# karpathy/minbpe

Measured on AMD Instinct MI355X. Metric: BPE merges/sec, higher is better.
Workload: dtype int32; 1 GPU; regex1g: RegexTokenizer.train, 1 GB synth seed 2, vocab 32000; mode=default, parallelism=single

## Files before the change

### minbpe_amd/csrc/kernels/k_chain.hip

```cpp
#include <hip/hip_runtime.h>
#include <stdint.h>

#include "../bpe_device.h"

namespace bpe {
namespace BPE_G {

constexpr uint32_t CH_EX_CAP = 2048;

__device__ __forceinline__ int chain_match(const uint32_t *pa, const uint32_t *pb, uint32_t K, uint32_t w0, uint32_t w1) {
    const uint32_t x = w0 & IDMASK, y = w1 & NWMASK;
    int hit = -1;
    for (uint32_t p = 0; p < K; p++)
        if (x == pa[p] && y == pb[p]) hit = (int)p;
    return (w0 == INVALID_WORD) ? -1 : hit;
}

constexpr uint32_t CH_DCAP = 1024;
constexpr uint32_t CH_SD = 2 * CH_DCAP + 2;
__device__ __forceinline__ void chain_slot_load(const AbArgs &A, const uint32_t t, uint4 (&rv)[MJ], uint4 &hv) {
    const int lane = lane_id();
    const uint32_t *src = A.b0 + (size_t)t * TILE2;
#pragma unroll
    for (int j = 0; j < MJ; j++) rv[j] = *reinterpret_cast<const uint4 *>(src + j * 256 + lane * 4);
// ... 6 lines not shown
                                                 const uint32_t *pa, const uint32_t *pb, const uint32_t *pb1,
                                                 const uint32_t K, const uint32_t z0, const uint32_t brep,
                                                 uint4 (&rv)[MJ], const uint4 hv,
                                                 const uint32_t *ph = nullptr, const uint32_t hm = 0,
                                                 const uint32_t tl_in = 0xFFFFFFFFu) {
    const int lane = lane_id();
    const uint32_t Tl = tl_in != 0xFFFFFFFFu ? tl_in : min(A.T, A.st->tlive);
    const uint32_t *src;
    const uint32_t meta = bcast(hv.w, 2);
    const uint32_t len = meta & 0x7FFFFFFFu, buf = meta >> 31;
    auto keep_header = [&]() {
        if (DENSE && (lane == 2 || lane == 3)) reinterpret_cast<uint4 *>(A.hdr_out)[2 * (size_t)t + (lane - 2)] = hv;
    };
    if (len == 0) {
        keep_header();
        return;
    }
    if (buf) {
        src = A.b1 + (size_t)t * TILE2;
#pragma unroll
        for (int j = 0; j < MJ; j++) rv[j] = *reinterpret_cast<const uint4 *>(src + j * 256 + lane * 4);
    }
    const uint32_t first = bcast(hv.x, 2);
    uint32_t halo0 = bcast(hv.x, 4), halo1 = bcast(hv.y, 4), halo2 = bcast(hv.z, 4);
    uint32_t prev2 = bcast(hv.x, 1), prev1 = bcast(hv.y, 1);
    uint32_t tprev = t - 1;
    uint32_t tnext = t + 1;
    {
        const uint32_t nlen = bcast(hv.w, 4) & 0x7FFFFFFFu, plen = bcast(hv.w, 0) & 0x7FFFFFFFu;
        if ((t + 1 < Tl && nlen < 3) || (t > 0 && plen < 2)) {
            uint32_t ctx[7] = {0, 0, 0, 0, 0, 0, 0};
            if (lane == 0) slot_context_walk(A.hdr_in, t, Tl, ctx);
            halo0 = bcast(ctx[0], 0);
            halo1 = bcast(ctx[1], 0);
            halo2 = bcast(ctx[2], 0);
            prev2 = bcast(ctx[3], 0);
            prev1 = bcast(ctx[4], 0);
            tprev = bcast(ctx[5], 0);
            tnext = bcast(ctx[6], 0);
        }
    }
    auto at = [&](int q, uint32_t own) -> uint32_t {
        const int d = q - (int)len;
        return d < 0 ? own : (d == 0 ? halo0 : (d == 1 ? halo1 : (d == 2 ? halo2 : INVALID_WORD)));
    };
    uint32_t x[MJ][4];
#pragma unroll
    for (int j = 0; j < MJ; j++) {
        const int q0 = j * 256 + lane * 4;
        if ((j + 1) * 256 <= (int)len) {
            x[j][0] = rv[j].x;
            x[j][1] = rv[j].y;
            x[j][2] = rv[j].z;
            x[j][3] = rv[j].w;
        } else {
            x[j][0] = at(q0 + 0, rv[j].x);
            x[j][1] = at(q0 + 1, rv[j].y);
            x[j][2] = at(q0 + 2, rv[j].z);
            x[j][3] = at(q0 + 3, rv[j].w);
        }
    }
    uint32_t tail[3];
#pragma unroll
    for (int i = 0; i < 3; i++) tail[i] = at(TILE2 + i, 0u);
    uint32_t rb[MJ], jc[MJ], valid[MJ];
#pragma unroll
    for (int j = 0; j < MJ; j++) {
        rb[j] = 0;
        jc[j] = 0;
    }
    uint32_t s = 0;
    uint32_t ia[MJ];
#pragma unroll
    for (int j = 0; j < MJ; j++) ia[j] = 0;
    uint32_t ip = 0;
    if (hm) {
        auto code = [&](uint32_t w) -> uint32_t {
            const uint32_t id = w & IDMASK;
            const uint32_t e = ph[(__umul24(id, hm) >> 8) & 255u];
            return (e >> 8) == id ? (e & 255u) : 0u;
        };
#pragma unroll
        for (int j = 0; j < MJ; j++) {
#pragma unroll
            for (int k = 0; k < 4; k++) ia[j] |= code(x[j][k]) << (8 * k);
        }
        ip = code(prev1);
    } else {
        for (uint32_t p = 0; p < K; p++) {
            const uint32_t a = pa[p];
#pragma unroll
            for (int j = 0; j < MJ; j++) {
#pragma unroll
                for (int k = 0; k < 4; k++) ia[j] |= ((x[j][k] & IDMASK) == a) ? (p + 1u) << (8 * k) : 0u;
            }
            ip = ((prev1 & IDMASK) == a) ? p + 1u : ip;
        }
    }
#pragma unroll
    for (int j = 0; j < MJ; j++) {
        const uint32_t up = (j < MJ - 1) ? lane_first(x[(j + 1) % MJ][0]) : tail[0];
        const uint32_t nxw = lane_next(x[j][0], up);
#pragma unroll
        for (int k = 0; k < 4; k++) {
            const uint32_t nxt = (k < 3) ? x[j][k + 1] : nxw;
            const uint32_t i = (ia[j] >> (8 * k)) & 255u;
            const uint32_t m = (uint32_t)((nxt & NWMASK) == pb1[i]);
            rb[j] |= m << k;
            jc[j] |= (m ? i : 0u) << (8 * k);
        }
    }
    s = (uint32_t)((prev1 != INVALID_WORD) & ((first & NWMASK) == pb1[ip]));
#pragma unroll
    for (int j = 0; j < MJ; j++) {
        const int nb = (int)len - (j * 256 + lane * 4);
        valid[j] = nb >= 4 ? 0xFu : (nb <= 0 ? 0u : ((1u << nb) - 1u));
    }
    uint32_t anyr = 0;
#pragma unroll
    for (int j = 0; j < MJ; j++) anyr |= rb[j] & valid[j];
    const bool sites = __any(anyr != 0) != 0;
    if (!sites && !s) {
        keep_header();
        return;
    }
    uint32_t mb[MJ], kb[MJ], ex[MJ], cnt[MJ];
#pragma unroll
    for (int j = 0; j < MJ; j++) {
        mb[j] = rb[j] & valid[j];
        const uint32_t upr = (j > 0) ? ((lane_last(rb[(j + MJ - 1) % MJ]) >> 3) & 1u) : s;
        const uint32_t mp = (uint32_t)dpp_mov<0x138>((int)upr, (int)((rb[j] >> 3) & 1u));
        kb[j] = ~((mb[j] << 1) | mp) & valid[j] & 0xFu;
        cnt[j] = (uint32_t)__popc(kb[j]);
    }
    uint32_t total = 0;
    if constexpr (MJ == 4) {
        const uint32_t i01 = wave_iscan_add(cnt[0] | (cnt[1] << 16));
        const uint32_t i23 = wave_iscan_add(cnt[2] | (cnt[3] << 16));
        const uint32_t t01 = lane_last(i01), t23 = lane_last(i23);
        const uint32_t tot0 = t01 & 0xFFFFu, tot1 = t01 >> 16, tot2 = t23 & 0xFFFFu, tot3 = t23 >> 16;
        ex[0] = (i01 & 0xFFFFu) - cnt[0];
        ex[1] = tot0 + (i01 >> 16) - cnt[1];
        ex[2] = tot0 + tot1 + (i23 & 0xFFFFu) - cnt[2];
        ex[3] = tot0 + tot1 + tot2 + (i23 >> 16) - cnt[3];
        total = tot0 + tot1 + tot2 + tot3;
    } else {
#pragma unroll
        for (int j = 0; j < MJ; j++) {
            const uint32_t inc = wave_iscan_add(cnt[j]);
            ex[j] = total + inc - cnt[j];
            total += lane_last(inc);
        }
    }
    uint32_t fstore = 0;
    if (!s) {
        uint32_t fc = 0x7FFFFFFFu;
#pragma unroll
        for (int j = 0; j < MJ; j++) {
            if (mb[j]) {
                const uint32_t k0 = (uint32_t)__ffs((int)mb[j]) - 1u;
                fc = min(fc, ex[j] + (uint32_t)__popc(kb[j] & ((1u << k0) - 1u)));
            }
        }
        fstore = (uint32_t)wave_min_i32((int)fc) & ~3u;
    }
#pragma unroll
    for (int j = 0; j < MJ; j++) {
        uint32_t o = ex[j];
#pragma unroll
        for (int k = 0; k < 4; k++) {
            if ((kb[j] >> k) & 1u) {
                const uint32_t w = x[j][k];
                const uint32_t z = z0 + ((jc[j] >> (8 * k)) & 255u) - 1u;
                out[o++] = ((mb[j] >> k) & 1u) ? (z | (w & (FLAG | WMASK))) : w;
            }
        }
    }
    __builtin_amdgcn_fence(__ATOMIC_RELEASE, "wavefront");
    __builtin_amdgcn_wave_barrier();
    __builtin_amdgcn_fence(__ATOMIC_ACQUIRE, "wavefront");
    {
        uint32_t *dst = (buf ? A.b1 : A.b0) + (size_t)t * TILE2;
        for (uint32_t i = fstore + (uint32_t)lane * 4; i < total; i += 256)
            *reinterpret_cast<uint4 *>(dst + i) = *reinterpret_cast<const uint4 *>(&out[i]);
    }
    if (lane == 0) {
        uint32_t h[8];
        h[0] = total > 0 ? out[0] : INVALID_WORD;
        h[1] = total > 1 ? out[1] : INVALID_WORD;
        h[2] = total > 2 ? out[2] : INVALID_WORD;
        h[3] = total | (buf << 31);
        h[4] = total > 1 ? out[total - 2] : INVALID_WORD;
        h[5] = total > 0 ? out[total - 1] : INVALID_WORD;
        h[6] = h[7] = 0;
        if (DENSE) {
            reinterpret_cast<uint4 *>(A.hdr_out)[2 * (size_t)t] = make_uint4(h[0], h[1], h[2], h[3]);
            reinterpret_cast<uint4 *>(A.hdr_out)[2 * (size_t)t + 1] = make_uint4(h[4], h[5], 0u, 0u);
        } else {
            stage_put<THROUGH>(A.stage + t, t, h);
            atomicOr(&A.smask[t >> 5], 1u << (t & 31));
        }
        if (total < 3 && t + 1 < Tl) A.st->gap = 1;
    }
    if (!sites) return;
    const uint32_t vc = A.vcap & 0xFFFFFFu;
    uint32_t cm2 = 0, ct0 = 0, ct1 = 0;
    if (bcast(mb[0], 0) & 1u) cm2 = (uint32_t)(chain_match(pa, pb, K, prev2, prev1) + 1);
    const uint32_t cm1 = s ? ip : 0u;
    if (bcast(mb[MJ - 1], 63) & 0xCu) {
        ct0 = (uint32_t)(chain_match(pa, pb, K, tail[0], tail[1]) + 1);
        ct1 = (uint32_t)(chain_match(pa, pb, K, tail[1], tail[2]) + 1);
    }
#pragma unroll
    for (int j = 0; j < MJ; j++) {
        if (!__any(mb[j] != 0)) continue;
        uint32_t upm1, dn0;
        if (j > 0) upm1 = lane_last(x[(j + MJ - 1) % MJ][3]);
        else upm1 = prev1;
        if (j < MJ - 1) dn0 = lane_first(x[(j + 1) % MJ][0]);
        else dn0 = tail[0];
        uint32_t W[7];
        W[0] = (uint32_t)dpp_mov<0x138>((int)upm1, (int)x[j][3]);
        W[1] = x[j][0];
        W[2] = x[j][1];
        W[3] = x[j][2];
        W[4] = x[j][3];
        W[5] = lane_next(x[j][0], dn0);
        W[6] = lane_next(x[j][1], (j < MJ - 1) ? lane_first(x[(j + 1) % MJ][1]) : tail[1]);
        const uint32_t lo_fill = (j > 0) ? (lane_last(jc[(j + MJ - 1) % MJ]) >> 16) : (cm2 | (cm1 << 8));
        const uint32_t hi_fill = (j < MJ - 1) ? (lane_first(jc[(j + 1) % MJ]) & 0xFFFFu) : (ct0 | (ct1 << 8));
        const uint32_t lo = (uint32_t)dpp_mov<0x138>((int)lo_fill, (int)(jc[j] >> 16));
        const uint32_t hi = lane_next(jc[j] & 0xFFFFu, hi_fill);
        const unsigned long long win = (unsigned long long)lo | ((unsigned long long)jc[j] << 16) | ((unsigned long long)hi << 48);
        if (mb[j] == 0) continue;
        uint32_t todo = mb[j];
#pragma unroll
        for (int si = 0; si < 2; si++) {
            if (todo == 0) continue;
            const uint32_t k = (uint32_t)__ffs((int)todo) - 1u;
            todo &= todo - 1u;
            const int q = j * 256 + lane * 4 + (int)k;
            const unsigned long long wk = win >> (8u * k);
            const uint32_t p = ((uint32_t)(wk >> 16) & 255u) - 1u;
            const int li = (int)((uint32_t)wk & 255u) - 1, ri = (int)((uint32_t)(wk >> 32) & 255u) - 1;
            const uint32_t Z = z0 + p;
            uint32_t *dl, *dr;
            if (DENSE) {
                dl = sd + p * CH_SD;
                dr = dl + CH_DCAP;
                atomicAdd(&dl[2 * CH_DCAP + 1], 1u);
            } else {
                if (A.removed) atomicAdd(&A.removed[(p * (uint32_t)CH_RMV + (t & (uint32_t)(CH_RMV - 1))) * REMOVED_STRIDE], 1u);
                dl = A.delta + delta_rep_off(p * (uint32_t)CH_RSTRIDE + (t & (brep - 1u)), vc);
                dr = dl + vc;
            }
            const bool k1 = (k & 1u) != 0, k2 = (k & 2u) != 0;
            const uint32_t wa = k2 ? (k1 ? W[4] : W[3]) : (k1 ? W[2] : W[1]);
            const uint32_t wt = word_weight(wa);
            const uint32_t Lw = k2 ? (k1 ? W[3] : W[2]) : (k1 ? W[1] : W[0]);
            if (!(wa & FLAG) && Lw != INVALID_WORD) {
                if (li != (int)p) {
                    const uint32_t Lseq = (li >= 0 && (uint32_t)li < p) ? z0 + (uint32_t)li : (Lw & IDMASK);
                    atomicAdd(&dl[Lseq], wt);
                    if (!DENSE || A.idx) {
                        const uint32_t Lfin = li >= 0 ? z0 + (uint32_t)li : (Lw & IDMASK);
                        index_add(A.idx, A.istride, t, Lfin, Z);
                        if (q == 0) index_add(A.idx, A.istride, tprev, Lfin, Z);
                    }
                }
            }
            const uint32_t R = k2 ? (k1 ? W[6] : W[5]) : (k1 ? W[4] : W[3]);
            if (!(R & FLAG)) {
                if (ri == (int)p) {
                    if (DENSE) atomicAdd(&dl[2 * CH_DCAP], wt);
                    else atomicAdd(&A.st->badj[p], wt);
                } else {
                    atomicAdd(&dr[(ri >= 0 && (uint32_t)ri < p) ? z0 + (uint32_t)ri : (R & IDMASK)], wt);
                }
                if (!DENSE || A.idx) {
                    const uint32_t y = ri >= 0 ? z0 + (uint32_t)ri : (R & IDMASK);
                    index_add(A.idx, A.istride, t, Z, y);
                    if (q + 2 >= (int)len) index_add(A.idx, A.istride, tnext, Z, y);
                }
            }
        }
    }
}

__device__ __forceinline__ void merge_aa_wave(uint32_t *scr, const uint32_t t, const AbArgs &A, const ChainAa &X, const uint32_t a,
                                              const uint32_t newid, const uint32_t Tl) {
    const int lane = lane_id();
    uint32_t *s_hdr = scr, *s_halo = scr + 8;
    uint4 hv6 = (lane & 1) ? make_uint4(INVALID_WORD, INVALID_WORD, 0u, 0u) : make_uint4(INVALID_WORD, INVALID_WORD, INVALID_WORD, 0u);
    {
        const long long hi = 2ll * (long long)t - 2 + lane;
        if (lane < 6 && hi >= 0 && hi < 2ll * (long long)A.T) hv6 = reinterpret_cast<const uint4 *>(A.hdr_in)[hi];
    }
    const uint32_t mi = bcast(hv6.w, 2);
    const int len = (int)(mi & 0x7FFFFFFFu);
    if (len == 0) return;
    const uint32_t cur = mi >> 31;
    const uint32_t *src = (cur ? A.b1 : A.b0) + (size_t)t * TILE2;
    const uint32_t first = bcast(hv6.x, 2);
    uint32_t halo0 = bcast(hv6.x, 4), halo1 = bcast(hv6.y, 4), halo2 = bcast(hv6.z, 4);
    uint32_t prev1 = bcast(hv6.y, 1);
    uint32_t tnext = t + 1;
    {
        const uint32_t nlen = bcast(hv6.w, 4) & 0x7FFFFFFFu, plen = bcast(hv6.w, 0) & 0x7FFFFFFFu;
        if ((t + 1 < Tl && nlen < 3) || (t > 0 && plen < 2)) {
            uint32_t ctx[7] = {0, 0, 0, 0, 0, 0, 0};
            if (lane == 0) slot_context_walk(A.hdr_in, t, Tl, ctx);
            halo0 = bcast(ctx[0], 0);
            halo1 = bcast(ctx[1], 0);
            halo2 = bcast(ctx[2], 0);
            prev1 = bcast(ctx[4], 0);
            tnext = bcast(ctx[6], 0);
        }
    }
    const uint32_t hw1 = bcast(hv6.y, 2), hw2 = bcast(hv6.z, 2), hl0 = bcast(hv6.x, 3), hl1 = bcast(hv6.y, 3);
    if (lane == 0) {
        s_hdr[0] = first;
        s_hdr[1] = hw1;
        s_hdr[2] = hw2;
        s_hdr[3] = mi;
        s_hdr[4] = hl0;
        s_hdr[5] = hl1;
        s_halo[0] = halo0;
        s_halo[1] = halo1;
        s_halo[2] = halo2;
    }
    SlotRaw raw;
    slot_raw_load<true>(raw, src, len);
    __builtin_amdgcn_fence(__ATOMIC_RELEASE, "wavefront");
    __builtin_amdgcn_wave_barrier();
    __builtin_amdgcn_fence(__ATOMIC_ACQUIRE, "wavefront");
    Tile tl;
    tile_from_slot<true>(tl, raw, len, s_halo);
    tile_rbits(tl, a, a);
    uint32_t s = (uint32_t)((prev1 != INVALID_WORD) & ((prev1 & IDMASK) == a) & ((first & NWMASK) == a));
    {
        const unsigned long long tag = ((unsigned long long)(X.epoch & EPOCH_MASK)) << 42;
        uint32_t sc = 0;
        bool failed = false;
        if (s) {
            uint32_t u = t;
            uint32_t mu = 0;
            while (u-- > 0) {
                mu = A.hdr_in[u].meta;
                if (mu & 0x7FFFFFFFu) break;
            }
            const int lu = (int)(mu & 0x7FFFFFFFu);
            const uint32_t *pu = ((mu >> 31) ? A.b1 : A.b0) + (size_t)u * TILE2;
            int ones = 0;
            bool open = true;
            uint32_t nextw = first;
            for (int base = lu - 1; base >= 0 && open; base -= 64) {
                const int q = base - lane;
                const uint32_t xq = (q >= 0) ? pu[q] : INVALID_WORD;
                uint32_t nx = (uint32_t)__shfl_up((int)xq, 1);
                if (lane == 0) nx = nextw;
                const bool r = (q >= 0) && ((xq & IDMASK) == a) && ((nx & NWMASK) == a);
                const unsigned long long zeros = __ballot(!r);
                if (zeros) {
                    ones += __ffsll((long long)zeros) - 1;
                    const int zl = __ffsll((long long)zeros) - 1;
                    open = (base - zl < 0);
                    break;
                }
                ones += 64;
                nextw = (uint32_t)__shfl((int)xq, 63);
            }
            if (!open || ones < lu) {
                sc = (uint32_t)(ones & 1);
            } else {
                uint32_t su = 0;
                bool got = false;
                for (uint32_t spins = 0; spins < LOOKBACK_SPINS; spins++) {
                    const unsigned long long d = desc_load(&X.sdesc[u]);
                    if ((d >> 42) == (tag >> 42) + (1ull << 20)) {
                        su = (uint32_t)(d & 1u);
                        got = true;
                        break;
                    }
                    __builtin_amdgcn_s_sleep(8);
                }
                failed = !got;
                sc = (uint32_t)(((lu - 1) & 1) == 0) ^ su;
            }
        }
        if (lane == 0) {
            desc_store(&X.sdesc[t], tag | (1ull << 62) | sc);
            if (failed) atomicExch(&A.st->status, ST_LOOKBACK);
        }
        s = sc;
    }
    {
        uint32_t anyr = s;
        const int q0 = lane * 4;
        const int nb = len + 1 - q0;
        const uint32_t keep = nb >= 4 ? 0xFu : (nb <= 0 ? 0u : ((1u << nb) - 1u));
        anyr |= tl.rb[0] & keep;
        if (len == TILE2) anyr |= (uint32_t)(((tl.tail[0] & IDMASK) == a) & ((tl.tail[1] & NWMASK) == a));
        if (!__any(anyr != 0)) return;
    }
    tile_lzscan<true>(tl, nullptr);
    uint32_t kept = 0;
    bool changed = false;
    uint32_t *dst = (cur ? A.b0 : A.b1) + (size_t)t * TILE2;
    tile_rewrite<true, true, 1, true>(tl, s, a, a, newid, dst, nullptr, A.delta, A.vcap, len, &kept, &changed, s_hdr, A.idx,
                                      A.istride, t, tnext, t);
    __builtin_amdgcn_fence(__ATOMIC_RELEASE, "wavefront");
    __builtin_amdgcn_wave_barrier();
    __builtin_amdgcn_fence(__ATOMIC_ACQUIRE, "wavefront");
    if (lane == 0 && changed) {
        uint32_t h[8];
        h[0] = kept > 0 ? s_hdr[0] : INVALID_WORD;
        h[1] = kept > 1 ? s_hdr[1] : INVALID_WORD;
        h[2] = kept > 2 ? s_hdr[2] : INVALID_WORD;
        h[3] = kept | ((cur ^ 1u) << 31);
        h[4] = kept > 1 ? s_hdr[4] : INVALID_WORD;
        h[5] = kept > 0 ? s_hdr[5] : INVALID_WORD;
        h[6] = h[7] = 0;
        stage_put<false>(A.stage + t, t, h);
        atomicOr(&A.smask[t >> 5], 1u << (t & 31));
        atomicAdd(&X.removed[(t & 255u) * REMOVED_STRIDE], (uint32_t)len - kept);
        if (kept < 3 && t + 1 < Tl) A.st->gap = 1;
    }
    __builtin_amdgcn_fence(__ATOMIC_RELEASE, "wavefront");
    __builtin_amdgcn_wave_barrier();
}

__device__ __forceinline__ uint32_t chain_hash_find(const uint32_t *pa, uint32_t K, uint32_t *tab) {
    if (K < 5) return 0u;
    const uint32_t lane = (uint32_t)lane_id(), half = lane >> 5, l = lane & 31u;
    const bool in = l < K;
    const uint32_t a = in ? pa[l] : 0u;
// ... 741 lines not shown
```

### minbpe_amd/csrc/kernels/k_slots2.hip

```cpp
#include <hip/hip_runtime.h>
#include <stdint.h>

#include "../bpe_device.h"

namespace bpe {
namespace BPE_G {



__global__ void __launch_bounds__(256)
k_slot2_init(SlotHdr *__restrict__ hdr, uint64_t T, DevState *st, int par, uint32_t which,
             const uint32_t *__restrict__ ids) {
    const uint64_t n = st->n[par];
    if (blockIdx.x == 0 && threadIdx.x == 0) {
        st->gap = 0;
        st->tlive = (uint32_t)min(T, (n + TILE2 - 1) / TILE2);
    }
    const uint64_t stride = (uint64_t)gridDim.x * blockDim.x;
    for (uint64_t t = (uint64_t)blockIdx.x * blockDim.x + threadIdx.x; t < T; t += stride) {
        const uint64_t b0 = t * TILE2;
        const uint32_t len = b0 >= n ? 0u : (uint32_t)min((uint64_t)TILE2, n - b0);
        SlotHdr h;
        h.w0 = len > 0 ? ids[b0] : INVALID_WORD;
        h.w1 = len > 1 ? ids[b0 + 1] : INVALID_WORD;
// ... 31 lines not shown
    for (uint32_t u = t; u-- > 0 && got < 2;) {
        const SlotHdr hh = hdr[u];
        const uint32_t lu = hh.meta & 0x7FFFFFFFu;
        if (lu == 0) continue;
        if (got == 0) {
            p1 = hh.l1;
            tp = u;
            got = 1;
            if (lu >= 2) {
                p2 = hh.l0;
                got = 2;
            }
        } else {
            p2 = hh.l1;
            got = 2;
        }
    }
    ctx[0] = h0;
    ctx[1] = h1;
    ctx[2] = h2;
    ctx[3] = p2;
    ctx[4] = p1;
    ctx[5] = tp;
    ctx[6] = tn;
}

__device__ __forceinline__ uint32_t bcast(uint32_t v, int srclane) {
    return (uint32_t)__builtin_amdgcn_readlane((int)v, srclane);
}

template <bool SPARSE, bool INDEXED, bool LDSD, bool THROUGH = false>
__device__ __forceinline__ void merge_ab_wave(uint32_t *__restrict__ out, uint32_t *__restrict__ sd, const uint32_t t,
                                              const AbArgs &A, const uint32_t a, const uint32_t b,
                                              const uint32_t tl_in = 0xFFFFFFFFu) {
    const int lane = lane_id();
    const uint32_t Tl = tl_in != 0xFFFFFFFFu ? tl_in : min(A.T, A.st->tlive);
    const uint32_t *src = A.b0 + (size_t)t * TILE2;
    uint4 rv[MJ];
#pragma unroll
    for (int j = 0; j < MJ; j++) rv[j] = *reinterpret_cast<const uint4 *>(src + j * 256 + lane * 4);
    uint4 hv = (lane & 1) ? make_uint4(INVALID_WORD, INVALID_WORD, 0u, 0u)
                          : make_uint4(INVALID_WORD, INVALID_WORD, INVALID_WORD, 0u);
    {
        const long long hi = 2ll * (long long)t - 2 + lane;
        if (lane < 6 && hi >= 0 && hi < 2ll * (long long)A.T) hv = reinterpret_cast<const uint4 *>(A.hdr_in)[hi];
    }
    const uint32_t meta = bcast(hv.w, 2);
    const uint32_t len = meta & 0x7FFFFFFFu, buf = meta >> 31;
    auto keep_header = [&]() {
        if (!SPARSE && (lane == 2 || lane == 3)) reinterpret_cast<uint4 *>(A.hdr_out)[2 * (size_t)t + (lane - 2)] = hv;
    };
    if (len == 0) {
        keep_header();
        return;
    }
    if (buf) {
        src = A.b1 + (size_t)t * TILE2;
#pragma unroll
        for (int j = 0; j < MJ; j++) rv[j] = *reinterpret_cast<const uint4 *>(src + j * 256 + lane * 4);
    }
    const uint32_t first = bcast(hv.x, 2);
    uint32_t halo0 = bcast(hv.x, 4), halo1 = bcast(hv.y, 4), halo2 = bcast(hv.z, 4);
    uint32_t prev2 = bcast(hv.x, 1), prev1 = bcast(hv.y, 1);
    uint32_t tprev = t - 1;
    uint32_t tnext = t + 1;
    {
        const uint32_t nlen = bcast(hv.w, 4) & 0x7FFFFFFFu, plen = bcast(hv.w, 0) & 0x7FFFFFFFu;
        if ((t + 1 < Tl && nlen < 3) || (t > 0 && plen < 2)) {
            uint32_t ctx[7] = {0, 0, 0, 0, 0, 0, 0};
            if (lane == 0) slot_context_walk(A.hdr_in, t, Tl, ctx);
            halo0 = bcast(ctx[0], 0);
            halo1 = bcast(ctx[1], 0);
            halo2 = bcast(ctx[2], 0);
            prev2 = bcast(ctx[3], 0);
            prev1 = bcast(ctx[4], 0);
            tprev = bcast(ctx[5], 0);
            tnext = bcast(ctx[6], 0);
        }
    }
    auto at = [&](int q, uint32_t own) -> uint32_t {
        const int d = q - (int)len;
        return d < 0 ? own : (d == 0 ? halo0 : (d == 1 ? halo1 : (d == 2 ? halo2 : INVALID_WORD)));
    };
    uint32_t x[MJ][4];
#pragma unroll
    for (int j = 0; j < MJ; j++) {
        const int q0 = j * 256 + lane * 4;
        if ((j + 1) * 256 <= (int)len) {
            x[j][0] = rv[j].x;
            x[j][1] = rv[j].y;
            x[j][2] = rv[j].z;
            x[j][3] = rv[j].w;
        } else {
            x[j][0] = at(q0 + 0, rv[j].x);
            x[j][1] = at(q0 + 1, rv[j].y);
            x[j][2] = at(q0 + 2, rv[j].z);
            x[j][3] = at(q0 + 3, rv[j].w);
        }
    }
    uint32_t tail[3];
#pragma unroll
    for (int i = 0; i < 3; i++) tail[i] = at(TILE2 + i, 0u);
    uint32_t rb[MJ], valid[MJ];
    uint32_t anyr = 0;
#pragma unroll
    for (int j = 0; j < MJ; j++) {
        const uint32_t up = (j < MJ - 1) ? lane_first(x[(j + 1) % MJ][0]) : tail[0];
        const uint32_t nx = lane_next(x[j][0], up);
        uint32_t r = 0;
#pragma unroll
        for (int k = 0; k < 4; k++) {
            const uint32_t nxt = (k < 3) ? x[j][k + 1] : nx;
            r |= (uint32_t)(((x[j][k] & IDMASK) == a) & ((nxt & NWMASK) == b)) << k;
        }
        const int nb = (int)len - (j * 256 + lane * 4);
        valid[j] = nb >= 4 ? 0xFu : (nb <= 0 ? 0u : ((1u << nb) - 1u));
        rb[j] = r;
        anyr |= r & valid[j];
    }
    const uint32_t s = (uint32_t)((prev1 != INVALID_WORD) & ((prev1 & IDMASK) == a) & ((first & NWMASK) == b));
    const bool sites = __any(anyr != 0) != 0;
    if (!sites && !s) {
        keep_header();
        return;
    }
    uint32_t mb[MJ], kb[MJ], ex[MJ], cnt[MJ];
#pragma unroll
    for (int j = 0; j < MJ; j++) {
        mb[j] = rb[j] & valid[j];
        const uint32_t upr = (j > 0) ? ((lane_last(rb[(j + MJ - 1) % MJ]) >> 3) & 1u) : s;
        const uint32_t mp = (uint32_t)dpp_mov<0x138>((int)upr, (int)((rb[j] >> 3) & 1u));
        kb[j] = ~((mb[j] << 1) | mp) & valid[j] & 0xFu;
        cnt[j] = (uint32_t)__popc(kb[j]);
    }
    uint32_t total = 0;
    if constexpr (MJ == 4) {
        const uint32_t i01 = wave_iscan_add(cnt[0] | (cnt[1] << 16));
        const uint32_t i23 = wave_iscan_add(cnt[2] | (cnt[3] << 16));
        const uint32_t t01 = lane_last(i01), t23 = lane_last(i23);
        const uint32_t tot0 = t01 & 0xFFFFu, tot1 = t01 >> 16, tot2 = t23 & 0xFFFFu, tot3 = t23 >> 16;
        ex[0] = (i01 & 0xFFFFu) - cnt[0];
        ex[1] = tot0 + (i01 >> 16) - cnt[1];
        ex[2] = tot0 + tot1 + (i23 & 0xFFFFu) - cnt[2];
        ex[3] = tot0 + tot1 + tot2 + (i23 >> 16) - cnt[3];
        total = tot0 + tot1 + tot2 + tot3;
    } else {
#pragma unroll
        for (int j = 0; j < MJ; j++) {
            const uint32_t inc = wave_iscan_add(cnt[j]);
            ex[j] = total + inc - cnt[j];
            total += lane_last(inc);
        }
    }
    uint32_t fstore = 0;
    if (!s) {
        uint32_t fc = 0x7FFFFFFFu;
#pragma unroll
        for (int j = 0; j < MJ; j++) {
            if (mb[j]) {
                const uint32_t k0 = (uint32_t)__ffs((int)mb[j]) - 1u;
                fc = min(fc, ex[j] + (uint32_t)__popc(kb[j] & ((1u << k0) - 1u)));
            }
        }
        fstore = (uint32_t)wave_min_i32((int)fc) & ~3u;
    }
#pragma unroll
    for (int j = 0; j < MJ; j++) {
        uint32_t o = ex[j];
#pragma unroll
        for (int k = 0; k < 4; k++) {
            if ((kb[j] >> k) & 1u) {
                const uint32_t w = x[j][k];
                out[o++] = ((mb[j] >> k) & 1u) ? (A.newid | (w & (FLAG | WMASK))) : w;
            }
        }
    }
    __builtin_amdgcn_fence(__ATOMIC_RELEASE, "wavefront");
    __builtin_amdgcn_wave_barrier();
    __builtin_amdgcn_fence(__ATOMIC_ACQUIRE, "wavefront");
    {
        uint32_t *dst = (buf ? A.b1 : A.b0) + (size_t)t * TILE2;
        for (uint32_t i = fstore + (uint32_t)lane * 4; i < total; i += 256)
            *reinterpret_cast<uint4 *>(dst + i) = *reinterpret_cast<const uint4 *>(&out[i]);
    }
    if (lane == 0) {
        uint32_t h[8];
        h[0] = total > 0 ? out[0] : INVALID_WORD;
        h[1] = total > 1 ? out[1] : INVALID_WORD;
        h[2] = total > 2 ? out[2] : INVALID_WORD;
        h[3] = total | (buf << 31);
        h[4] = total > 1 ? out[total - 2] : INVALID_WORD;
        h[5] = total > 0 ? out[total - 1] : INVALID_WORD;
        h[6] = h[7] = 0;
        if (!SPARSE) {
            reinterpret_cast<uint4 *>(A.hdr_out)[2 * (size_t)t] = make_uint4(h[0], h[1], h[2], h[3]);
            reinterpret_cast<uint4 *>(A.hdr_out)[2 * (size_t)t + 1] = make_uint4(h[4], h[5], 0u, 0u);
        } else {
            stage_put<THROUGH>(A.stage + t, t, h);
            atomicOr(&A.smask[t >> 5], 1u << (t & 31));
        }
        if (LDSD) atomicAdd(&sd[2 * LDSD_CAP + 1], len - total);
        else if (A.removed) atomicAdd(&A.removed[(t & 255u) * REMOVED_STRIDE], len - total);
        if (total < 3 && t + 1 < Tl) A.st->gap = 1;
    }
    if (!sites) return;
    if (!A.delta) return;
    const uint32_t nrep = 1u << (A.vcap >> 24);
    const uint32_t vc = A.vcap & 0xFFFFFFu;
    uint32_t *dl = A.delta + delta_rep_off(t & (nrep - 1), vc);
    uint32_t *dr = dl + vc;
    uint32_t adj = 0;
#pragma unroll
    for (int j = 0; j < MJ; j++) {
        if (!__any(mb[j] != 0)) continue;
        uint32_t upm2, upm1, dn0, dn1, dn2;
        if (j > 0) {
            upm2 = lane_last(x[(j + MJ - 1) % MJ][2]);
            upm1 = lane_last(x[(j + MJ - 1) % MJ][3]);
        } else {
            upm2 = prev2;
            upm1 = prev1;
        }
        if (j < MJ - 1) {
            dn0 = lane_first(x[(j + 1) % MJ][0]);
            dn1 = lane_first(x[(j + 1) % MJ][1]);
            dn2 = lane_first(x[(j + 1) % MJ][2]);
        } else {
            dn0 = tail[0];
            dn1 = tail[1];
            dn2 = tail[2];
        }
        uint32_t W[9];
        W[0] = (uint32_t)dpp_mov<0x138>((int)upm2, (int)x[j][2]);
        W[1] = (uint32_t)dpp_mov<0x138>((int)upm1, (int)x[j][3]);
        W[2] = x[j][0];
        W[3] = x[j][1];
        W[4] = x[j][2];
        W[5] = x[j][3];
        W[6] = lane_next(x[j][0], dn0);
        W[7] = lane_next(x[j][1], dn1);
        W[8] = lane_next(x[j][2], dn2);
        if (mb[j] == 0) continue;
        uint32_t todo = mb[j];
#pragma unroll
        for (int si = 0; si < 2; si++) {
            if (todo == 0) continue;
            const uint32_t k = (uint32_t)__ffs((int)todo) - 1u;
            todo &= todo - 1u;
            const int q = j * 256 + lane * 4 + (int)k;
            const bool k1 = (k & 1u) != 0, k2 = (k & 2u) != 0;
            auto wsel = [&](int o) -> uint32_t { return k2 ? (k1 ? W[o + 3] : W[o + 2]) : (k1 ? W[o + 1] : W[o]); };
            const uint32_t wa = wsel(2);
            const uint32_t wt = word_weight(wa);
            const uint32_t Lw = wsel(1), LL = wsel(0);
            if (!(wa & FLAG) && Lw != INVALID_WORD) {
                const bool ltail = ((LL & IDMASK) == a) & ((Lw & NWMASK) == b);
                if (!ltail) {
                    if (LDSD) atomicAdd(&sd[Lw & IDMASK], wt);
                    else atomicAdd(&dl[Lw & IDMASK], wt);
                    if (INDEXED) {
                        index_add(A.idx, A.istride, t, Lw & IDMASK, A.newid);
                        if (q == 0) index_add(A.idx, A.istride, tprev, Lw & IDMASK, A.newid);
                    }
                }
            }
            const uint32_t R = wsel(4), RR = wsel(5);
            if (!(R & FLAG)) {
                const bool rsite = ((R & IDMASK) == a) & ((RR & NWMASK) == b);
                if (rsite) adj += wt;
                else if (LDSD) atomicAdd(&sd[LDSD_CAP + (R & IDMASK)], wt);
                else atomicAdd(&dr[R & IDMASK], wt);
                if (INDEXED) {
                    const uint32_t y = rsite ? A.newid : (R & IDMASK);
                    index_add(A.idx, A.istride, t, A.newid, y);
                    if (q + 2 >= (int)len) index_add(A.idx, A.istride, tnext, A.newid, y);
                }
            }
        }
    }
    if (__any(adj != 0)) {
        adj = wave_sum_u32(adj);
        if (lane == 0) {
            if (LDSD) atomicAdd(&sd[2 * LDSD_CAP], adj);
            else atomicAdd(&A.st->adj, adj);
        }
    }
}

__device__ __forceinline__ void ldsd_clear(uint32_t *sd) {
    for (uint32_t i = threadIdx.x; i < 2 * LDSD_CAP + 2; i += MT) sd[i] = 0;
    __syncthreads();
}
__device__ __forceinline__ void ldsd_flush(const uint32_t *sd, const AbArgs &A) {
    __syncthreads();
    const uint32_t nrep = 1u << (A.vcap >> 24);
    const uint32_t vc = A.vcap & 0xFFFFFFu;
    if (A.delta) {
        uint32_t *g = A.delta + delta_rep_off(blockIdx.x & (nrep - 1), vc);
        const uint32_t lim = min(vc, (uint32_t)LDSD_CAP);
        for (uint32_t i = threadIdx.x; i < lim; i += MT) {
            const uint32_t l = sd[i], r = sd[LDSD_CAP + i];
            if (l) atomicAdd(&g[i], l);
            if (r) atomicAdd(&g[vc + i], r);
        }
    }
    if (threadIdx.x == 0) {
        const uint32_t adj = sd[2 * LDSD_CAP], rem = sd[2 * LDSD_CAP + 1];
        if (adj) atomicAdd(&A.st->adj, adj);
        if (rem && A.removed) atomicAdd(&A.removed[(blockIdx.x & 255u) * REMOVED_STRIDE], rem);
    }
}

template <bool INDEXED>
__global__ void __launch_bounds__(MT, INDEXED ? 5 : 7)
k_merge_ab_dense(AbArgs A) {
    __shared__ __attribute__((aligned(16))) uint32_t s_out[MT / 64][TILE2];
    const DevState *st = A.st;
    if (blockIdx.x == 0 && threadIdx.x == 0) *A.dirty_n = 0;
    const uint32_t t = blockIdx.x * (MT / 64) + wave_id();
    if (t >= A.T || st->status) return;
    if (!st->found) {
        if (t == 0 && lane_id() == 0) A.st->status = ST_INTERNAL;
        return;
    }
    const uint32_t a = (uint32_t)st->a, b = (uint32_t)st->b;
    if (a == b) return;
    merge_ab_wave<false, INDEXED, false>(s_out[wave_id()], nullptr, t, A, a, b);
}
template <bool INDEXED>
__global__ void __launch_bounds__(MT, 5)
k_merge_ab_dense_early(AbArgs A) {
    __shared__ __attribute__((aligned(16))) uint32_t s_out[MT / 64][TILE2];
    __shared__ uint32_t s_delta[2 * LDSD_CAP + 2];
    const DevState *st = A.st;
    if (blockIdx.x == 0 && threadIdx.x == 0) *A.dirty_n = 0;
    if (st->status) return;
    if (!st->found) {
        if (blockIdx.x == 0 && threadIdx.x == 0) A.st->status = ST_INTERNAL;
        return;
    }
    const uint32_t a = (uint32_t)st->a, b = (uint32_t)st->b;
    if (a == b) return;
    ldsd_clear(s_delta);
    const uint32_t nw = gridDim.x * (MT / 64);
    const uint32_t Tl = min(A.T, st->tlive);
    for (uint32_t t = blockIdx.x * (MT / 64) + wave_id(); t < A.T; t += nw)
        merge_ab_wave<false, INDEXED, true>(s_out[wave_id()], s_delta, t, A, a, b, Tl);
    ldsd_flush(s_delta, A);
}

#ifndef AB_SPARSE_WAVES
#define AB_SPARSE_WAVES 4
#endif
template <bool LDSD>
__global__ void __launch_bounds__(MT, AB_SPARSE_WAVES)
k_merge_ab_sparse(AbArgs A) {
    __shared__ __attribute__((aligned(16))) uint32_t s_out[MT / 64][TILE2];
    __shared__ uint32_t s_delta[LDSD ? 2 * LDSD_CAP + 2 : 1];
    const DevState *st = A.st;
    if (blockIdx.x == 0 && threadIdx.x == 0) *A.dirty_n = 0;
    if (st->status) return;
    if (!st->found) {
        if (blockIdx.x == 0 && threadIdx.x == 0) A.st->status = ST_INTERNAL;
        return;
    }
    const uint32_t a = (uint32_t)st->a, b = (uint32_t)st->b;
    if (a == b) return;
    const uint32_t n = st->ncand;
    const uint32_t nw = gridDim.x * (MT / 64);
    if (LDSD) {
        if (blockIdx.x * (MT / 64) >= n) return;
        ldsd_clear(s_delta);
    }
    const uint32_t Tl = min(A.T, st->tlive);
    for (uint32_t i = blockIdx.x * (MT / 64) + wave_id(); i < n; i += nw)
        merge_ab_wave<true, true, LDSD>(s_out[wave_id()], s_delta, A.cand[i], A, a, b, Tl);
    if (LDSD) ldsd_flush(s_delta, A);
}


__device__ __forceinline__ void merge_aa_tile(const uint32_t t, const AaArgs &A, const uint32_t a, const uint32_t Tl) {
    __shared__ int s_wave[MT / 64];
    __shared__ uint32_t s_wsum[MT / 64];
    __shared__ uint32_t s_ctx[8];
    __shared__ uint32_t s_hdr[8];
    const uint32_t b = a;
    uint4 hv6 = (lane_id() & 1) ? make_uint4(INVALID_WORD, INVALID_WORD, 0u, 0u) : make_uint4(INVALID_WORD, INVALID_WORD, INVALID_WORD, 0u);
    {
        const long long hi = 2ll * (long long)t - 2 + lane_id();
        if (lane_id() < 6 && hi >= 0 && hi < 2ll * (long long)A.T) hv6 = reinterpret_cast<const uint4 *>(A.hdr_in)[hi];
    }
    SlotHdr hme;
    hme.w0 = bcast(hv6.x, 2);
    hme.w1 = bcast(hv6.y, 2);
    hme.w2 = bcast(hv6.z, 2);
    hme.meta = bcast(hv6.w, 2);
    hme.l0 = bcast(hv6.x, 3);
    hme.l1 = bcast(hv6.y, 3);
    hme.pad0 = hme.pad1 = 0;
    const uint32_t mi = hme.meta;
    const int len = (int)(mi & 0x7FFFFFFFu);
    uint4 *out4 = reinterpret_cast<uint4 *>(A.hdr_out + t);
    auto keep_header = [&]() {
        if (!A.stage) {
            out4[0] = make_uint4(hme.w0, hme.w1, hme.w2, hme.meta);
            out4[1] = make_uint4(hme.l0, hme.l1, 0u, 0u);
        }
    };
    if (len == 0) {
        if (threadIdx.x == 0) keep_header();
        return;
    }
    const uint32_t cur = mi >> 31;
    const uint32_t *src = (cur ? A.b1 : A.b0) + (size_t)t * TILE2;
    const uint32_t nlen = bcast(hv6.w, 4) & 0x7FFFFFFFu, plen = bcast(hv6.w, 0) & 0x7FFFFFFFu;
    const uint32_t nh0 = bcast(hv6.x, 4), nh1 = bcast(hv6.y, 4), nh2 = bcast(hv6.z, 4), pp2 = bcast(hv6.x, 1), pp1 = bcast(hv6.y, 1);
    if (threadIdx.x == 0) {
        if ((t + 1 < Tl && nlen < 3) || (t > 0 && plen < 2)) {
            slot_context_walk(A.hdr_in, t, Tl, s_ctx);
        } else {
            s_ctx[0] = nh0;
            s_ctx[1] = nh1;
            s_ctx[2] = nh2;
            s_ctx[3] = pp2;
            s_ctx[4] = pp1;
            s_ctx[5] = t - 1;
            s_ctx[6] = t + 1;
        }
        s_hdr[0] = hme.w0;
        s_hdr[1] = hme.w1;
        s_hdr[2] = hme.w2;
// ... 267 lines not shown
```

Measured before the change: 56930 merges/s.

## Compact merge sites into dense lane list for delta accumulation in dense paths

In the dense (non-sparse) variants of the chain and slot kernels, merge-site positions are packed after the compacted output in the scratch buffer using a wave prefix scan. The neighbour-delta and index updates then iterate over this compacted site list with one lane per site, reading neighbours from the rewritten output instead of reconstructing windows via DPP across all slots. This targets divergence and idle lanes when sites are sparse, at the cost of an extra scan, more scratch writes, and per-pair ballot loops to count removed sites.

```diff
diff --git a/minbpe_amd/csrc/kernels/k_chain.hip b/minbpe_amd/csrc/kernels/k_chain.hip
--- a/minbpe_amd/csrc/kernels/k_chain.hip
+++ b/minbpe_amd/csrc/kernels/k_chain.hip
@@ -182,6 +182,19 @@
             total += lane_last(inc);
         }
     }
+    uint32_t sx[MJ], nsites = 0;
+    if constexpr (DENSE) {
+        uint32_t pk = 0;
+#pragma unroll
+        for (int j = 0; j < MJ; j++) pk |= (uint32_t)__popc(mb[j]) << (8 * j);
+        const uint32_t inc = wave_iscan_add(pk);
+        const uint32_t tl = lane_last(inc);
+#pragma unroll
+        for (int j = 0; j < MJ; j++) {
+            sx[j] = nsites + ((inc >> (8 * j)) & 255u) - (uint32_t)__popc(mb[j]);
+            nsites += (tl >> (8 * j)) & 255u;
+        }
+    }
     uint32_t fstore = 0;
     if (!s) {
         uint32_t fc = 0x7FFFFFFFu;
@@ -203,6 +216,21 @@
                 const uint32_t w = x[j][k];
                 const uint32_t z = z0 + ((jc[j] >> (8 * k)) & 255u) - 1u;
                 out[o++] = ((mb[j] >> k) & 1u) ? (z | (w & (FLAG | WMASK))) : w;
+            }
+        }
+    }
+    const uint32_t nl = len - total - s;
+    if constexpr (DENSE) {
+#pragma unroll
+        for (int j = 0; j < MJ; j++) {
+            if (mb[j]) {
+                const uint32_t k0 = (uint32_t)__ffs((int)mb[j]) - 1u;
+                if (sx[j] < nl) out[total + sx[j]] = ex[j] + (uint32_t)__popc(kb[j] & ((1u << k0) - 1u));
+                const uint32_t m1 = mb[j] & (mb[j] - 1u);
+                if (m1) {
+                    const uint32_t k1 = (uint32_t)__ffs((int)m1) - 1u;
+                    if (sx[j] + 1u < nl) out[total + sx[j] + 1u] = ex[j] + (uint32_t)__popc(kb[j] & ((1u << k1) - 1u));
+                }
             }
         }
     }
@@ -233,6 +261,65 @@
         if (total < 3 && t + 1 < Tl) A.st->gap = 1;
     }
     if (!sites) return;
+    if constexpr (DENSE) {
+        const uint32_t wfirst = (uint32_t)__builtin_amdgcn_readfirstlane((int)out[0]);
+        const uint32_t wlast = (uint32_t)__builtin_amdgcn_readfirstlane((int)out[total - 1]);
+        uint32_t lctx = prev1, rctx = INVALID_WORD;
+        if ((wfirst & IDMASK) >= z0) {
+            if (s) {
+                lctx = z0 + ip - 1u;
+            } else {
+                const int c = chain_match(pa, pb, K, prev2, prev1);
+                if (c >= 0) lctx = z0 + (uint32_t)c;
+            }
+        }
+        if ((wlast & IDMASK) >= z0) {
+            const bool span = nsites != nl;
+            const uint32_t R = span ? halo1 : halo0, RR = span ? halo2 : halo1;
+            const int c = chain_match(pa, pb, K, R, RR);
+            rctx = c >= 0 ? ((z0 + (uint32_t)c) | (R & FLAG)) : R;
+        }
+        for (uint32_t i0 = 0; i0 < nsites; i0 += 64) {
+            const uint32_t i = i0 + (uint32_t)lane;
+            const bool act = i < nsites;
+            uint32_t p = 0xFFFFFFFFu;
+            if (act) {
+                const uint32_t o = i < nl ? out[total + i] : total - 1u;
+                const uint32_t wz = out[o];
+                const uint32_t wt = word_weight(wz);
+                const uint32_t Z = wz & IDMASK;
+                p = Z - z0;
+                const uint32_t Lin = out[max(o, 1u) - 1u], Rin = out[min(o + 1u, total - 1u)];
+                const uint32_t Lw = o > 0 ? Lin : lctx;
+                const uint32_t R = o + 1u < total ? Rin : rctx;
+                uint32_t *dl = sd + p * CH_SD, *dr = dl + CH_DCAP;
+                if (!(wz & FLAG) && Lw != INVALID_WORD) {
+                    const uint32_t lid = Lw & IDMASK;
+                    if (lid != Z) {
+                        atomicAdd(&dl[lid > Z ? pb[lid - z0] : lid], wt);
+                        if (A.idx) {
+                            index_add(A.idx, A.istride, t, lid, Z);
+                            if (o == 0 && !s) index_add(A.idx, A.istride, tprev, lid, Z);
+                        }
+                    }
+                }
+                if (!(R & FLAG)) {
+                    const uint32_t rid = R & IDMASK;
+                    if (rid == Z) atomicAdd(&dl[2 * CH_DCAP], wt);
+                    else atomicAdd(&dr[rid > Z ? pa[rid - z0] : rid], wt);
+                    if (A.idx) {
+                        index_add(A.idx, A.istride, t, Z, rid);
+                        if (o + 1u == total) index_add(A.idx, A.istride, tnext, Z, rid);
+                    }
+                }
+            }
+            for (uint32_t q = 0; q < K; q++) {
+                const uint32_t c = (uint32_t)__popcll(__ballot(p == q));
+                if (lane == 0 && c) atomicAdd(&sd[q * CH_SD + 2 * CH_DCAP + 1], c);
+            }
+        }
+        return;
+    }
     const uint32_t vc = A.vcap & 0xFFFFFFu;
     uint32_t cm2 = 0, ct0 = 0, ct1 = 0;
     if (bcast(mb[0], 0) & 1u) cm2 = (uint32_t)(chain_match(pa, pb, K, prev2, prev1) + 1);
@@ -274,16 +361,9 @@
             const uint32_t p = ((uint32_t)(wk >> 16) & 255u) - 1u;
             const int li = (int)((uint32_t)wk & 255u) - 1, ri = (int)((uint32_t)(wk >> 32) & 255u) - 1;
             const uint32_t Z = z0 + p;
-            uint32_t *dl, *dr;
-            if (DENSE) {
-                dl = sd + p * CH_SD;
-                dr = dl + CH_DCAP;
-                atomicAdd(&dl[2 * CH_DCAP + 1], 1u);
-            } else {
-                if (A.removed) atomicAdd(&A.removed[(p * (uint32_t)CH_RMV + (t & (uint32_t)(CH_RMV - 1))) * REMOVED_STRIDE], 1u);
-                dl = A.delta + delta_rep_off(p * (uint32_t)CH_RSTRIDE + (t & (brep - 1u)), vc);
-                dr = dl + vc;
-            }
+            if (A.removed) atomicAdd(&A.removed[(p * (uint32_t)CH_RMV + (t & (uint32_t)(CH_RMV - 1))) * REMOVED_STRIDE], 1u);
+            uint32_t *dl = A.delta + delta_rep_off(p * (uint32_t)CH_RSTRIDE + (t & (brep - 1u)), vc);
+            uint32_t *dr = dl + vc;
             const bool k1 = (k & 1u) != 0, k2 = (k & 2u) != 0;
             const uint32_t wa = k2 ? (k1 ? W[4] : W[3]) : (k1 ? W[2] : W[1]);
             const uint32_t wt = word_weight(wa);
@@ -292,26 +372,18 @@
                 if (li != (int)p) {
                     const uint32_t Lseq = (li >= 0 && (uint32_t)li < p) ? z0 + (uint32_t)li : (Lw & IDMASK);
                     atomicAdd(&dl[Lseq], wt);
-                    if (!DENSE || A.idx) {
-                        const uint32_t Lfin = li >= 0 ? z0 + (uint32_t)li : (Lw & IDMASK);
-                        index_add(A.idx, A.istride, t, Lfin, Z);
-                        if (q == 0) index_add(A.idx, A.istride, tprev, Lfin, Z);
-                    }
+                    const uint32_t Lfin = li >= 0 ? z0 + (uint32_t)li : (Lw & IDMASK);
+                    index_add(A.idx, A.istride, t, Lfin, Z);
+                    if (q == 0) index_add(A.idx, A.istride, tprev, Lfin, Z);
                 }
             }
             const uint32_t R = k2 ? (k1 ? W[6] : W[5]) : (k1 ? W[4] : W[3]);
             if (!(R & FLAG)) {
-                if (ri == (int)p) {
-                    if (DENSE) atomicAdd(&dl[2 * CH_DCAP], wt);
-                    else atomicAdd(&A.st->badj[p], wt);
-                } else {
-                    atomicAdd(&dr[(ri >= 0 && (uint32_t)ri < p) ? z0 + (uint32_t)ri : (R & IDMASK)], wt);
-                }
-                if (!DENSE || A.idx) {
-                    const uint32_t y = ri >= 0 ? z0 + (uint32_t)ri : (R & IDMASK);
-                    index_add(A.idx, A.istride, t, Z, y);
-                    if (q + 2 >= (int)len) index_add(A.idx, A.istride, tnext, Z, y);
-                }
+                if (ri == (int)p) atomicAdd(&A.st->badj[p], wt);
+                else atomicAdd(&dr[(ri >= 0 && (uint32_t)ri < p) ? z0 + (uint32_t)ri : (R & IDMASK)], wt);
+                const uint32_t y = ri >= 0 ? z0 + (uint32_t)ri : (R & IDMASK);
+                index_add(A.idx, A.istride, t, Z, y);
+                if (q + 2 >= (int)len) index_add(A.idx, A.istride, tnext, Z, y);
             }
         }
     }
diff --git a/minbpe_amd/csrc/kernels/k_slots2.hip b/minbpe_amd/csrc/kernels/k_slots2.hip
--- a/minbpe_amd/csrc/kernels/k_slots2.hip
+++ b/minbpe_amd/csrc/kernels/k_slots2.hip
@@ -207,6 +207,19 @@
             total += lane_last(inc);
         }
     }
+    uint32_t sx[MJ], nsites = 0;
+    if constexpr (!SPARSE) {
+        uint32_t pk = 0;
+#pragma unroll
+        for (int j = 0; j < MJ; j++) pk |= (uint32_t)__popc(mb[j]) << (8 * j);
+        const uint32_t inc = wave_iscan_add(pk);
+        const uint32_t tl = lane_last(inc);
+#pragma unroll
+        for (int j = 0; j < MJ; j++) {
+            sx[j] = nsites + ((inc >> (8 * j)) & 255u) - (uint32_t)__popc(mb[j]);
+            nsites += (tl >> (8 * j)) & 255u;
+        }
+    }
     uint32_t fstore = 0;
     if (!s) {
         uint32_t fc = 0x7FFFFFFFu;
@@ -227,6 +240,21 @@
             if ((kb[j] >> k) & 1u) {
                 const uint32_t w = x[j][k];
                 out[o++] = ((mb[j] >> k) & 1u) ? (A.newid | (w & (FLAG | WMASK))) : w;
+            }
+        }
+    }
+    const uint32_t nl = len - total - s;
+    if constexpr (!SPARSE) {
+#pragma unroll
+        for (int j = 0; j < MJ; j++) {
+            if (mb[j]) {
+                const uint32_t k0 = (uint32_t)__ffs((int)mb[j]) - 1u;
+                if (sx[j] < nl) out[total + sx[j]] = ex[j] + (uint32_t)__popc(kb[j] & ((1u << k0) - 1u));
+                const uint32_t m1 = mb[j] & (mb[j] - 1u);
+                if (m1) {
+                    const uint32_t k1 = (uint32_t)__ffs((int)m1) - 1u;
+                    if (sx[j] + 1u < nl) out[total + sx[j] + 1u] = ex[j] + (uint32_t)__popc(kb[j] & ((1u << k1) - 1u));
+                }
             }
         }
     }
@@ -265,6 +293,50 @@
     uint32_t *dl = A.delta + delta_rep_off(t & (nrep - 1), vc);
     uint32_t *dr = dl + vc;
     uint32_t adj = 0;
+    if constexpr (!SPARSE) {
+        const uint32_t wfirst = (uint32_t)__builtin_amdgcn_readfirstlane((int)out[0]);
+        const uint32_t wlast = (uint32_t)__builtin_amdgcn_readfirstlane((int)out[total - 1]);
+        uint32_t lctx = prev1, rctx = INVALID_WORD;
+        if ((wfirst & IDMASK) == A.newid) {
+            if (s || (((prev2 & IDMASK) == a) & ((prev1 & NWMASK) == b))) lctx = A.newid;
+        }
+        if ((wlast & IDMASK) == A.newid) {
+            const bool span = nsites != nl;
+            const uint32_t R = span ? halo1 : halo0, RR = span ? halo2 : halo1;
+            rctx = (((R & IDMASK) == a) & ((RR & NWMASK) == b)) ? (A.newid | (R & FLAG)) : R;
+        }
+        for (uint32_t i0 = 0; i0 < nsites; i0 += 64) {
+            const uint32_t i = i0 + (uint32_t)lane;
+            if (i >= nsites) continue;
+            const uint32_t o = i < nl ? out[total + i] : total - 1u;
+            const uint32_t wz = out[o];
+            const uint32_t wt = word_weight(wz);
+            const uint32_t Lin = out[max(o, 1u) - 1u], Rin = out[min(o + 1u, total - 1u)];
+            const uint32_t Lw = o > 0 ? Lin : lctx;
+            const uint32_t R = o + 1u < total ? Rin : rctx;
+            if (!(wz & FLAG) && Lw != INVALID_WORD) {
+                const uint32_t lid = Lw & IDMASK;
+                if (lid != A.newid) {
+                    if (LDSD) atomicAdd(&sd[lid], wt);
+                    else atomicAdd(&dl[lid], wt);
+                    if (INDEXED) {
+                        index_add(A.idx, A.istride, t, lid, A.newid);
+                        if (o == 0 && !s) index_add(A.idx, A.istride, tprev, lid, A.newid);
+                    }
+                }
+            }
+            if (!(R & FLAG)) {
+                const uint32_t rid = R & IDMASK;
+                if (rid == A.newid) adj += wt;
+                else if (LDSD) atomicAdd(&sd[LDSD_CAP + rid], wt);
+                else atomicAdd(&dr[rid], wt);
+                if (INDEXED) {
+                    index_add(A.idx, A.istride, t, A.newid, rid);
+                    if (o + 1u == total) index_add(A.idx, A.istride, tnext, A.newid, rid);
+                }
+            }
+        }
+    } else {
 #pragma unroll
     for (int j = 0; j < MJ; j++) {
         if (!__any(mb[j] != 0)) continue;
@@ -332,6 +404,7 @@
                 }
             }
         }
+    }
     }
     if (__any(adj != 0)) {
         adj = wave_sum_u32(adj);
```

New measurement: 56870 merges/s, median of 2. About the same (-0.1%).
